# ouguangjun/Leg-KILO

Measured on NVIDIA H100. Metric: LiDAR point-iterations/sec through the ESKF point-to-plane update, higher is better.
Workload: dtype f64

## Files before the change

leg-kilo_b200/csrc/lk_fused.cu:

```cuda
#include "lk_insert.cuh"
#include "lk_kernels.h"
#include "lk_obs.cuh"
#include "lk_pass.cuh"
#include "lk_predict.cuh"
#include "lk_solve.cuh"

namespace lk {

namespace {

#define FT(slot) do { if (a.trace && threadIdx.x == 0 && (slot) < 32) a.trace[(size_t)blockIdx.x * 32 + (slot)] = gtime(); } while (0)
#define FTI(slot) do { if (it_global < 3) FT(slot); } while (0)
#define FTS(slot) do { if (a.trace && blockIdx.x == 0 && threadIdx.x == 0 && k < 64) a.trace[(size_t)gridDim.x * 32 + (size_t)k * 8 + (slot)] = gtime(); } while (0)
#ifndef LK_HOP_TRACE
#define LK_HOP_TRACE 0
#endif
#define FT_HOPS() ((LK_HOP_TRACE && a.trace && it_global < 3) \
                       ? a.trace + (size_t)gridDim.x * 32 + 64 * 8 + (size_t)blockIdx.x * 16 + it_global * LL_HOP_SLOTS : nullptr)

constexpr int BLOCK = FB;
constexpr int WARPS = BLOCK / 32;

struct PredictScratch {
    double F[900];
    double T[900];
    double Ps[900];
    ObsScratch obs;
};

template <bool HOT>
struct FusedSmemT {
    BlockFilter f;
    ScanConst sc;
    double slice[WARPS * 32];
    double clk[2];
    union {
        PredictScratch pr;
        PassSmem<BLOCK, HOT> pass;
    } u;
};
typedef FusedSmemT<true> FusedSmem;

struct FusedSmemIns {
    FusedSmemT<false> base;
    WarpTile wt[WARPS];
    MapDev md;
    Globals g;
};

__device__ __noinline__ void fused_insert_phase2(FusedSmemIns* si, const uint32_t* touched, const int* iroot, const DevPoint* ipts,
                                                 int* pend, uint32_t n_touched, uint32_t n_bucket) {
    const int lane = threadIdx.x & 31, warp = threadIdx.x >> 5;
    MapDev md = si->md;
    WarpTile* wt = si->wt + warp;
    for (uint32_t t = blockIdx.x * (uint32_t)WARPS + (uint32_t)warp; t < n_touched; t += gridDim.x * (uint32_t)WARPS)
        warp_insert_root_scan(md, si->g, wt, __ldcg(&touched[t]), iroot, ipts, n_bucket, pend, lane);
}

static_assert(sizeof(PredictScratch) <= sizeof(((PassSmem<BLOCK, true>*)0)->tile) &&
                  sizeof(PredictScratch) <= sizeof(((PassSmem<BLOCK, false>*)0)->tile),
              "predict scratch must not reach the mbarriers");
static_assert(sizeof(FusedSmemIns) <= 227 * 1024, "one block per SM");
static_assert(sizeof(FusedSmem) + 1024 <= 132 * 1024, "the batch-of-one kernel's stack frames must fit in L1");

int carveout_percent(size_t smem, int dev) {
    int per_sm = 0, per_block = 0;
    cudaDeviceGetAttribute(&per_sm, cudaDevAttrMaxSharedMemoryPerMultiprocessor, dev);
    cudaDeviceGetAttribute(&per_block, cudaDevAttrReservedSharedMemoryPerBlock, dev);
    if (per_sm <= 0) return 100;
    const size_t need = smem + (size_t)per_block;
    const int pct = (int)((need * 100 + (size_t)per_sm - 1) / (size_t)per_sm);
    return pct < 100 ? pct : 100;
}

template <class SM>
__device__ __noinline__ void fused_predict(SM* sm, const double* Q, double dtc, double dt) {
    if (dtc != 0.0) {
        build_F(sm->u.pr.F, sm->f.x, dtc);
        cov_predict(sm->f.P, sm->u.pr.F, sm->u.pr.T, sm->u.pr.Ps, Q, dtc);
    }
    if (dt != 0.0) {
        if (threadIdx.x == 0) state_predict(sm->f.x, dt);
    }
    fence_proxy_async();
    __syncthreads();
}

template <class SM>
__device__ __noinline__ void fused_drain_queue(SM* sm, const FusedArgs& a, uint32_t& mi, double t_bucket) {
    bool drained = false;
    while (mi < a.n_meas) {
        const double ts = a.imu ? a.imu[mi].stamp : a.kin[mi].stamp;
        if (!(ts < t_bucket)) break;
        block_predict_to(&sm->f, sm->clk, ts, sm->u.pr.F, sm->u.pr.T, sm->u.pr.Ps, a.Q);
        if (a.imu) block_obs_imu<BLOCK>(&sm->f, &sm->u.pr.obs, a.imu + mi, &a.ecfg, a.gravity, a.acc_norm);
        else block_obs_kinimu<BLOCK>(&sm->f, &sm->u.pr.obs, a.kin + mi, &a.ecfg, a.gravity, a.acc_norm);
        if (threadIdx.x == 0) sm->clk[1] = ts;
        __syncthreads();
        ++mi;
        drained = true;
    }
    if (drained) {
        fence_proxy_async();
        __syncthreads();
    }
}

__device__ __forceinline__ float4 world_out(const double* X, double pix, double piy, double piz, bool updated) {
    float4 o;
    o.x = (float)(X[0] * pix + X[1] * piy + X[2] * piz + X[9]);
    o.y = (float)(X[3] * pix + X[4] * piy + X[5] * piz + X[10]);
    o.z = (float)(X[6] * pix + X[7] * piy + X[8] * piz + X[11]);
    o.w = updated ? 255.0f : 0.0f;
    return o;
}

template <class SM>
__device__ __forceinline__ void store_state(SM* sm, const FusedArgs& a, uint32_t n_eff) {
    const int tid = threadIdx.x;
    if (tid < 36) a.x[(size_t)a.scan * 36 + tid] = sm->f.x[tid];
    if (tid < 2) reinterpret_cast<double*>(a.clk + a.scan)[tid] = sm->clk[tid];
    if (tid == 0) {
        a.n_eff[a.scan] = n_eff;
        *a.status = (*reinterpret_cast<volatile uint32_t*>(a.ll.stall) ? 1u : 0u) | (*reinterpret_cast<volatile uint32_t*>(&lk_stall_note[0]) ? 2u : 0u);
    }
}

typedef PassSmem<BLOCK, true> PassHot;
typedef PassSmem<BLOCK, false> PassNodes;
constexpr size_t FIN_GS_BYTES = (size_t)LL_MAX_GROUPS * 32 * sizeof(double);
constexpr uint32_t FIN_STAGE = (uint32_t)((sizeof(PassHot::tile) - FIN_GS_BYTES) / (3 * sizeof(double)));
static_assert(offsetof(PredictScratch, F) == 0 && offsetof(PassHot, tile) == 0 && offsetof(PassNodes, tile) == 0,
              "the group sums and the staging area start at the tiles");
static_assert(FIN_GS_BYTES + 3 * sizeof(double) * FIN_STAGE <= sizeof(PassHot::tile) &&
                  sizeof(PassHot::tile) <= sizeof(PassNodes::tile) && sizeof(PassHot::tile) <= offsetof(PassHot, bar),
              "the finishers' staging area must stay inside the tiles, clear of the mbarriers");

template <class SM>
__device__ __noinline__ void fused_finish(SM* sm, const FusedArgs& a, const StepInit& in, uint32_t n_chunks, uint32_t it_global,
                                          bool updated, bool dep_waited) {
    const int tid = threadIdx.x;
    const uint32_t fi = blockIdx.x - n_chunks, nf = gridDim.x - n_chunks;
    if (!dep_waited) asm volatile("griddepcontrol.wait;" ::: "memory");
    constexpr int U = 8;
    const uint32_t step = nf * BLOCK;
    const uint32_t first = in.pt_begin + fi * BLOCK + tid;
    double* st = reinterpret_cast<double*>(reinterpret_cast<unsigned char*>(&sm->u) + FIN_GS_BYTES);
    const uint32_t n_pts = first < in.pt_end ? (in.pt_end - first + step - 1) / step : 0u;
    const uint32_t n_st = a.pts_copy ? 0u : min(n_pts, (FIN_STAGE - (uint32_t)tid + BLOCK - 1) / BLOCK);
    for (uint32_t j0 = 0; j0 < n_st; j0 += U) {
        float4 q[U];
#pragma unroll
        for (int u = 0; u < U; ++u)
            if (j0 + u < n_st) q[u] = __ldcg(a.pts + first + (j0 + u) * step);
#pragma unroll
        for (int u = 0; u < U; ++u)
            if (j0 + u < n_st) {
                PointCtx p;
                imu_point(q[u], a.g, p);
                const uint32_t l = (j0 + u) * BLOCK + tid;
                st[l] = p.pix;
                st[FIN_STAGE + l] = p.piy;
                st[2 * FIN_STAGE + l] = p.piz;
            }
    }
    ll_sum_chunk_rows<WARPS>(a.ll, it_global & 1u, a.epoch + it_global, n_chunks, sm->u.pr.F, sm->f.acc);
    FTI(3 + it_global * 4);
    const uint32_t n = block_solve_state(&sm->f);
    FTI(4 + it_global * 4);
    if (n > 0) {
        updated = true;
        if (tid == 0) sm->clk[1] = in.t_bucket;
    }
    for (uint32_t j = 0; j < n_st; ++j) {
        const uint32_t l = j * BLOCK + tid;
        a.world[first + j * step] = world_out(sm->f.x, st[l], st[FIN_STAGE + l], st[2 * FIN_STAGE + l], updated);
    }
    const float4* pts = a.pts;
    if (a.pts_copy) {
        __threadfence();
        pts = a.pts_copy;
    }
    for (uint32_t i0 = first + n_st * step; i0 < in.pt_end; i0 += U * step) {
        float4 q[U];
#pragma unroll
        for (int u = 0; u < U; ++u)
            if (i0 + u * step < in.pt_end) q[u] = __ldcg(pts + i0 + u * step);
#pragma unroll
        for (int u = 0; u < U; ++u)
            if (i0 + u * step < in.pt_end) {
                PointCtx p;
                imu_point(q[u], a.g, p);
                a.world[i0 + u * step] = world_out(sm->f.x, p.pix, p.piy, p.piz, updated);
            }
    }
    FT(20);
    if (n > 0) cov_prep(&sm->f, BLOCK);
    __syncthreads();
    for (uint32_t e = fi * BLOCK + tid; e < 900; e += nf * BLOCK)
        a.P[(size_t)a.scan * 900 + e] = n > 0 ? cov_entry(&sm->f, (int)e) : sm->f.P[e];
    FT(21);
    if (fi == 0) store_state(sm, a, n);
    FT(22);
}

template <bool INL> struct InlineSel { typedef FusedInline type; };
template <> struct InlineSel<false> { typedef FusedNoInline type; };

__device__ __forceinline__ void grid_sync(const FusedArgs& a, uint32_t& sync_idx) {
    __threadfence();
    __syncthreads();
    if (threadIdx.x < 32) (void)ll_allreduce(a.ll, sync_idx & 1u, a.epoch + sync_idx, blockIdx.x, gridDim.x, 0.0, (int)threadIdx.x);
    ++sync_idx;
    __syncthreads();
    __threadfence();
    fence_proxy_async_global();
}

template <bool OBS, bool INL, bool INS>
__global__ void __launch_bounds__(BLOCK, 1) k_scan_fused(const __grid_constant__ FusedArgs a,
                                                         const __grid_constant__ typename InlineSel<INL>::type inl) {
    extern __shared__ __align__(16) unsigned char smem_raw[];
    FusedSmemT<!INS>* sm = reinterpret_cast<FusedSmemT<!INS>*>(smem_raw);
    const int tid = threadIdx.x, lane = tid & 31, warp = tid >> 5;
    const uint32_t scan = a.scan;
    const bool finisher = blockIdx.x + a.finishers >= gridDim.x;
    asm volatile("griddepcontrol.launch_dependents;" ::: "memory");
    FT(0);
    {
        const double* Pin;
        const double* xin;
        const double* cin;
        if constexpr (INL) { Pin = inl.P; xin = inl.x; cin = inl.clk; }
        else { Pin = a.P_in + (size_t)scan * 900; xin = a.x_in + (size_t)scan * 36; cin = reinterpret_cast<const double*>(a.clk_in + scan); }
        if (a.slim_p && !finisher && (a.finishers || blockIdx.x != 0)) {
            if (tid < 180) sm->f.P[(tid / 6) * 30 + tid % 6] = Pin[(tid / 6) * 30 + tid % 6];
        } else {
            for (int e = tid; e < 900; e += BLOCK) sm->f.P[e] = Pin[e];
        }
        if (tid < 36) sm->f.x[tid] = xin[tid];
        if (tid < 2) sm->clk[tid] = cin[tid];
    }
    if constexpr (INS) {
        FusedSmemIns* si = reinterpret_cast<FusedSmemIns*>(smem_raw);
        WarpTile* wt = si->wt + warp;
        if (lane == 0) {
            mbar_init(&wt->bar, 1);
            wt->phase = 0;
        }
        if (tid == 0) si->md = a.md;
        if (tid < (int)(sizeof(Globals) / 4)) reinterpret_cast<uint32_t*>(&si->g)[tid] = reinterpret_cast<const uint32_t*>(&a.g)[tid];
    }
    pass_init(&sm->u.pass);
    FT(1);
    uint32_t n_eff_total = 0;
    uint32_t phase = 0;
    uint32_t it_global = 0;
    uint32_t cslot = 0;
    uint32_t mi = 0;
    bool dep_waited = false;

    for (uint32_t k = 0; k < a.n_steps; ++k) {
        StepInit in;
        if constexpr (INL) in = inl.steps[k];
        else in = a.inits[(size_t)k * a.batch + scan];
        if (!in.active) continue;
        const uint32_t n_chunks = in.chunk_end - in.chunk_begin;
        const uint32_t my_start = in.pt_begin + blockIdx.x * (uint32_t)BLOCK;
        const uint32_t my_count = blockIdx.x < n_chunks ? min((uint32_t)BLOCK, in.pt_end - my_start) : 0u;
        float4 pre = make_float4(0.f, 0.f, 0.f, 0.f);
        if ((uint32_t)tid < my_count) pre = __ldg(a.pts + my_start + tid);
        FTS(0);
        if constexpr (OBS) fused_drain_queue(sm, a, mi, in.t_bucket);
        FTS(1);
        const double dtc = in.t_bucket - sm->clk[1];
        const double dt = in.t_bucket - sm->clk[0];
        if (dtc != 0.0 || dt != 0.0) fused_predict(sm, a.Q, dtc, dt);
        if (tid == 0) sm->clk[0] = in.t_bucket;
        FTS(2);
        bool updated = false, cov_pending = false;
        uint32_t n_last = 0;
        LaneCache lc;
        lc.have = 0;
        const bool more_steps = k + 1 < a.n_steps;
        for (int it = 0; it < a.iters; ++it, ++it_global) {
            scan_const_from(&sm->f, &sm->sc);
            __syncthreads();
            double acc[32];
#pragma unroll
            for (int i = 0; i < 32; ++i) acc[i] = 0.0;
            if (!a.lane_cache && lc.have == 2) lc.have = 1;
            points_pass<BLOCK, INS>(&sm->u.pass, phase, my_count, sm->sc, a.mv, a.g, lc, pre,
                                    [&](uint32_t, const Row& row) { accumulate_row(row, acc); });
            FTI(14 + it_global);
            const double tot = warp_transpose_sum(acc, lane);
            sm->slice[warp * 32 + lane] = tot;
            __syncthreads();
            FTI(2 + it_global * 4);
            if (it == 0) FTS(3);
            const bool last = it == a.iters - 1;
            if (!OBS && !INS && a.finishers && last) {
                if (finisher) {
                    fused_finish(sm, a, in, n_chunks, it_global, updated, dep_waited);
                } else {
                    if (!dep_waited) asm volatile("griddepcontrol.wait;" ::: "memory");
                    if (a.pts_copy) {
                        if ((uint32_t)tid < my_count) a.pts_copy[my_start + tid] = pre;
                        __threadfence();
                        __syncthreads();
                    }
                    if (warp == 0) {
                        double v = 0.0;
#pragma unroll
                        for (int w = 0; w < WARPS; ++w) v += sm->slice[w * 32 + lane];
                        ll_publish_row(a.ll, it_global & 1u, a.epoch + it_global, blockIdx.x, v, lane);
                    }
                }
                FT(31);
                return;
            }
            if (warp == 0) {
                double v = 0.0;
#pragma unroll
                for (int w = 0; w < WARPS; ++w) v += sm->slice[w * 32 + lane];
                if (!dep_waited) {
                    FT(23);
                    asm volatile("griddepcontrol.wait;" ::: "memory");
                    FT(24);
                }
                sm->f.acc[lane] = ll_allreduce(a.ll, it_global & 1u, a.epoch + it_global, blockIdx.x, n_chunks, v, lane, FT_HOPS(),
                                               a.finishers, it_global >= 2);
            }
            dep_waited = true;
            __syncthreads();
            FTI(3 + it_global * 4);
            if (it == 0) FTS(4);
            const uint32_t n = block_solve_state(&sm->f);
            FTI(4 + it_global * 4);
            if (n > 0) {
                updated = true;
                if (tid == 0) sm->clk[1] = in.t_bucket;
                if (last) cov_pending = INS || more_steps || blockIdx.x == 0;
            }
            n_last = n;
        }
        n_eff_total += n_last;
        FTS(5);
        if constexpr (!INS) {
            if ((uint32_t)tid < my_count) a.world[my_start + tid] = world_out(sm->f.x, lc.pix, lc.piy, lc.piz, updated);
            FT(20);
            if (cov_pending) block_cov_update<BLOCK>(&sm->f);
        } else {
            if (cov_pending) block_cov_update<BLOCK>(&sm->f);
            __syncthreads();
            scan_const_from(&sm->f, &sm->sc);
            __syncthreads();
            MapDev md = a.md;
            const uint32_t n_bucket = in.pt_end - in.pt_begin;
            if ((uint32_t)tid < my_count) {
                DevPoint p;
                make_insert_point(lc.pix, lc.piy, lc.piz, lc.pbx, lc.pby, lc.pbz, sm->sc, a.g, p);
                const uint32_t li = my_start + tid - in.pt_begin;
                a.ipts[li] = p;
                float4 o;
                o.x = (float)p.pw[0]; o.y = (float)p.pw[1]; o.z = (float)p.pw[2];
                o.w = updated ? 255.0f : 0.0f;
                a.world[my_start + tid] = o;
                a.iroot[li] = insert_register_point(md, a.g, p, a.pend, a.touched, &a.ins_counters[cslot]);
            }
            grid_sync(a, it_global);
            FTS(6);
            {
                const uint32_t n_touched = __ldcg(&a.ins_counters[cslot]);
                if (blockIdx.x == 0 && tid == 0) a.ins_counters[cslot ^ 1u] = 0;
                fused_insert_phase2(reinterpret_cast<FusedSmemIns*>(smem_raw), a.touched, a.iroot, a.ipts, a.pend, n_touched, n_bucket);
                cslot ^= 1u;
            }
            grid_sync(a, it_global);
            FTS(7);
        }
    }
    FT(30);
    if (blockIdx.x == 0) {
        if (!dep_waited) asm volatile("griddepcontrol.wait;" ::: "memory");
        __syncthreads();
        for (int e = tid; e < 900; e += BLOCK) a.P[(size_t)scan * 900 + e] = sm->f.P[e];
        store_state(sm, a, n_eff_total);
    }
    FT(31);
}

template <bool OBS, bool INL, bool INS>
cudaError_t launch_one(const FusedArgs& a, const FusedInline* inl, uint32_t grid, cudaStream_t s, int mode) {
    auto kern = k_scan_fused<OBS, INL, INS>;
    constexpr size_t SMEM = INS ? sizeof(FusedSmemIns) : sizeof(FusedSmem);
    static PerDeviceOnce once;
    if (once.first()) {
        int dev = 0;
        cudaGetDevice(&dev);
        cudaError_t e = cudaFuncSetAttribute(kern, cudaFuncAttributeMaxDynamicSharedMemorySize, (int)SMEM);
        if (e != cudaSuccess) return e;
        e = cudaFuncSetAttribute(kern, cudaFuncAttributePreferredSharedMemoryCarveout, carveout_percent(SMEM, dev));
        if (e != cudaSuccess) return e;
    }
    typename InlineSel<INL>::type local_inl;
    const typename InlineSel<INL>::type* ip;
    if constexpr (INL) ip = inl;
    else { local_inl.unused = 0; ip = &local_inl; }
    if (mode == FUSED_LAUNCH_COOPERATIVE) {
        void* params[] = {(void*)&a, (void*)ip};
        return cudaLaunchCooperativeKernel((const void*)kern, dim3(grid), dim3(BLOCK), params, SMEM, s);
    }
    cudaLaunchConfig_t cfg = {};
    cfg.gridDim = dim3(grid);
    cfg.blockDim = dim3(BLOCK);
    cfg.dynamicSmemBytes = SMEM;
    cfg.stream = s;
    cudaLaunchAttribute at[1];
    at[0].id = cudaLaunchAttributeProgrammaticStreamSerialization;
    at[0].val.programmaticStreamSerializationAllowed = 1;
    cfg.attrs = at;
    cfg.numAttrs = mode == FUSED_LAUNCH_PDL ? 1 : 0;
    return cudaLaunchKernelEx(&cfg, kern, a, *ip);
}

}

size_t fused_smem_bytes() { return sizeof(FusedSmem); }

int fused_read_stall(uint32_t out[8]) {
    if (cudaMemcpyFromSymbol(out, lk_stall_note, 32) != cudaSuccess) return -1;
    if (out[0]) {
        const uint32_t z[8] = {0, 0, 0, 0, 0, 0, 0, 0};
        cudaMemcpyToSymbol(lk_stall_note, z, 32);
    }
    return 0;
}

int fused_max_blocks(int device) {
    static int cached[64];
    static bool have[64];
    if (device >= 0 && device < 64 && have[device]) return cached[device];
    int sms = 0;
    cudaDeviceGetAttribute(&sms, cudaDevAttrMultiProcessorCount, device);
    int n = sms < LL_MAX_CHUNKS ? sms : LL_MAX_CHUNKS;
    if (device >= 0 && device < 64) { cached[device] = n; have[device] = true; }
    return n;
}

cudaError_t launch_scan_fused(const FusedArgs& a, const FusedInline* inl, uint32_t grid, cudaStream_t s, int mode) {
    const bool obs = a.n_meas > 0;
    if (a.insert) {
        if (inl) return cudaErrorInvalidValue;
        return obs ? launch_one<true, false, true>(a, inl, grid, s, mode) : launch_one<false, false, true>(a, inl, grid, s, mode);
    }
    if (obs) return inl ? launch_one<true, true, false>(a, inl, grid, s, mode) : launch_one<true, false, false>(a, inl, grid, s, mode);
    return inl ? launch_one<false, true, false>(a, inl, grid, s, mode) : launch_one<false, false, false>(a, inl, grid, s, mode);
}

}
```

leg-kilo_b200/csrc/lk_llsync.cuh:

```cuda
#pragma once
#include <cuda_runtime.h>
#include <stdint.h>

#include "lk_async.cuh"

namespace lk {

constexpr int LK_GROUP = 8;
constexpr int LL_ROW = 32;
constexpr int LL_MAX_CHUNKS = 160;
constexpr int LL_MAX_GROUPS = (LL_MAX_CHUNKS + LK_GROUP - 1) / LK_GROUP;
constexpr int LL_REPLICAS = 4;
constexpr int LL_COPIES = LL_REPLICAS + 1;
constexpr int LL_MAX_FINISHERS = 24;

struct LLView {
    ulonglong2* chunk_rows;
    ulonglong2* group_rows;
    uint32_t* stall;
    uint32_t* acks;
};
constexpr size_t LL_ROWS_BYTES = (size_t)2 * (LL_MAX_CHUNKS + LL_COPIES * LL_MAX_GROUPS) * LL_ROW * sizeof(ulonglong2);
constexpr size_t LL_BYTES = LL_ROWS_BYTES + 64 + 2 * LL_MAX_FINISHERS * sizeof(uint32_t);
constexpr uint32_t LL_SPIN_LIMIT = 1u << 23;
constexpr int LL_HOP_SLOTS = 5;

__device__ __forceinline__ void ll_store(ulonglong2* p, double v, uint32_t tag) {
    const unsigned long long b = (unsigned long long)__double_as_longlong(v);
    const unsigned long long t = (unsigned long long)tag << 32;
    const unsigned long long w0 = (b & 0xffffffffull) | t, w1 = (b >> 32) | t;
    asm volatile("st.relaxed.gpu.global.v2.u64 [%0], {%1, %2};" ::"l"(p), "l"(w0), "l"(w1) : "memory");
}

__device__ __forceinline__ void ll_give_up(uint32_t* stall, uint32_t tag, uint32_t r0, uint32_t n, int lane) {
    if (atomicCAS(stall, 0u, 1u) == 0u) {
        stall[1] = blockIdx.x; stall[2] = tag; stall[3] = r0; stall[4] = n; stall[5] = (uint32_t)lane;
        __threadfence();
    }
}

template <int N, bool KEEP, int SPLIT = N>
__device__ __forceinline__ double ll_sum_rows(const ulonglong2* rows, uint32_t r0, uint32_t n, uint32_t tag, int lane,
                                              uint32_t* stall, uint32_t& rounds, double first = 0.0, bool have_first = false,
                                              double* hi = nullptr) {
    static_assert(N <= 32, "one bit per row");
    const ulonglong2* p = rows + (size_t)r0 * LL_ROW + lane;
    unsigned long long w0[N], w1[N];
    const unsigned long long want = ((unsigned long long)tag << 32);
    uint32_t spins = 0;
    if constexpr (!KEEP) {
        bool all;
        do {
#pragma unroll
            for (int k = 0; k < N; ++k)
                if ((uint32_t)k < n && !(have_first && k == 0))
                    asm volatile("ld.relaxed.gpu.global.v2.u64 {%0, %1}, [%2];" : "=l"(w0[k]), "=l"(w1[k]) : "l"(p + (size_t)k * LL_ROW));
            all = true;
#pragma unroll
            for (int k = 0; k < N; ++k)
                if ((uint32_t)k < n && !(have_first && k == 0))
                    all = all && ((w0[k] & 0xffffffff00000000ull) == want) && ((w1[k] & 0xffffffff00000000ull) == want);
            ++spins;
            if (!all && ((spins & 0xfffu) == 0u)) {
                if (spins >= LL_SPIN_LIMIT || *reinterpret_cast<volatile uint32_t*>(stall) != 0u) {
                    ll_give_up(stall, tag, r0, n, lane);
                    break;
                }
            }
        } while (!all);
    } else {
        uint32_t todo = (n >= 32u ? 0xffffffffu : (1u << n) - 1u) & (have_first ? ~1u : ~0u);
        while (true) {
#pragma unroll
            for (int k = 0; k < N; ++k)
                if ((todo >> k) & 1u)
                    asm volatile("ld.relaxed.gpu.global.v2.u64 {%0, %1}, [%2];" : "=l"(w0[k]), "=l"(w1[k]) : "l"(p + (size_t)k * LL_ROW));
#pragma unroll
            for (int k = 0; k < N; ++k)
                if (((todo >> k) & 1u) && ((w0[k] & 0xffffffff00000000ull) == want) && ((w1[k] & 0xffffffff00000000ull) == want))
                    todo &= ~(1u << k);
            ++spins;
            if (todo == 0u) break;
            if ((spins & 0xfffu) == 0u) {
                if (spins >= LL_SPIN_LIMIT || *reinterpret_cast<volatile uint32_t*>(stall) != 0u) {
                    ll_give_up(stall, tag, r0, n, lane);
                    break;
                }
            }
        }
    }
    rounds = spins;
    double s = 0.0;
#pragma unroll
    for (int k = 0; k < SPLIT; ++k)
        if ((uint32_t)k < n) {
            const double v = (have_first && k == 0) ? first : __longlong_as_double((long long)((w0[k] & 0xffffffffull) | (w1[k] << 32)));
            s += v;
        }
    if constexpr (SPLIT < N) {
        double s2 = 0.0;
#pragma unroll
        for (int k = SPLIT; k < N; ++k)
            if ((uint32_t)k < n) s2 += __longlong_as_double((long long)((w0[k] & 0xffffffffull) | (w1[k] << 32)));
        *hi = s2;
    }
    return s;
}

__device__ __forceinline__ void ll_wait_acks(const uint32_t* acks, uint32_t fin, uint32_t tag, int lane, uint32_t* stall) {
    uint32_t spins = 0;
    bool mine = (uint32_t)lane >= fin;
    while (!__all_sync(0xffffffffu, mine)) {
        if (!mine) {
            uint32_t w;
            asm volatile("ld.acquire.gpu.global.u32 %0, [%1];" : "=r"(w) : "l"(acks + lane) : "memory");
            mine = w == tag;
        }
        if ((++spins & 0xfffu) == 0u && (spins >= LL_SPIN_LIMIT || *reinterpret_cast<volatile uint32_t*>(stall) != 0u)) {
            ll_give_up(stall, tag, 0, fin, lane);
            break;
        }
    }
}

__device__ __forceinline__ double ll_allreduce(const LLView& ll, uint32_t parity, uint32_t tag, uint32_t b, uint32_t n_chunks,
                                               double v, int lane, unsigned long long* hops = nullptr, uint32_t fin = 0,
                                               bool acks_due = false) {
    constexpr size_t COPY = (size_t)LL_MAX_GROUPS * LL_ROW;
    ulonglong2* crows = ll.chunk_rows + (size_t)parity * LL_MAX_CHUNKS * LL_ROW;
    ulonglong2* grows = ll.group_rows + (size_t)parity * LL_COPIES * COPY;
    uint32_t* acks = ll.acks + (size_t)parity * LL_MAX_FINISHERS;
    const uint32_t n_groups = (n_chunks + LK_GROUP - 1) / LK_GROUP;
    uint32_t r1 = 0, r2 = 0;
    if (b < n_chunks) {
        if ((b % LK_GROUP) == 0) {
            if (hops && lane == 0) hops[0] = gtime();
            const uint32_t n = min((uint32_t)LK_GROUP, n_chunks - b);
            const double s = ll_sum_rows<LK_GROUP, false>(crows, b, n, tag, lane, ll.stall, r1, v, true);
            if (hops && lane == 0) hops[1] = gtime();
            ulonglong2* g = grows + (size_t)(b / LK_GROUP) * LL_ROW + lane;
            if (fin && acks_due) ll_wait_acks(acks, fin, tag - 2u, lane, ll.stall);
#pragma unroll
            for (int r = 0; r < LL_REPLICAS; ++r) ll_store(g + (size_t)r * COPY, s, tag);
            if (fin) ll_store(g + (size_t)LL_REPLICAS * COPY, s, tag);
            if (hops && lane == 0) hops[2] = gtime();
        } else {
            ll_store(crows + (size_t)b * LL_ROW + lane, v, tag);
            if (hops && lane == 0) hops[0] = gtime();
        }
    }
    const bool finisher = fin && b >= n_chunks;
    const double t = ll_sum_rows<LL_MAX_GROUPS, true>(grows + (size_t)(finisher ? LL_REPLICAS : b % LL_REPLICAS) * COPY, 0, n_groups,
                                                      tag, lane, ll.stall, r2);
    if (finisher) {
        __syncwarp();
        if (lane == 0) asm volatile("st.release.gpu.global.u32 [%0], %1;" ::"l"(acks + (b - n_chunks)), "r"(tag) : "memory");
    }
    if (hops) {
        r1 = __reduce_max_sync(0xffffffffu, r1);
        r2 = __reduce_max_sync(0xffffffffu, r2);
        if (lane == 0) {
            hops[3] = gtime();
            hops[4] = (unsigned long long)r1 | ((unsigned long long)r2 << 32);
        }
    }
    return t;
}

__device__ __forceinline__ void ll_publish_row(const LLView& ll, uint32_t parity, uint32_t tag, uint32_t b, double v, int lane) {
    ll_store(ll.chunk_rows + ((size_t)parity * LL_MAX_CHUNKS + b) * LL_ROW + lane, v, tag);
}

template <int NWARPS>
__device__ __forceinline__ void ll_sum_chunk_rows(const LLView& ll, uint32_t parity, uint32_t tag, uint32_t n_chunks, double* gs,
                                                  double* out) {
    const int tid = threadIdx.x, lane = tid & 31, warp = tid >> 5;
    const ulonglong2* crows = ll.chunk_rows + (size_t)parity * LL_MAX_CHUNKS * LL_ROW;
    const uint32_t n_groups = (n_chunks + LK_GROUP - 1) / LK_GROUP;
    for (uint32_t g = 2u * (uint32_t)warp; g < n_groups; g += 2u * NWARPS) {
        uint32_t rounds;
        double hi;
        gs[g * 32 + lane] = ll_sum_rows<2 * LK_GROUP, true, LK_GROUP>(crows, g * LK_GROUP, min(2u * LK_GROUP, n_chunks - g * LK_GROUP),
                                                                       tag, lane, ll.stall, rounds, 0.0, false, &hi);
        if (g + 1 < n_groups) gs[(g + 1) * 32 + lane] = hi;
    }
    __syncthreads();
    if (tid < 32) {
        double t = 0.0;
        for (uint32_t g = 0; g < n_groups; ++g) t += gs[g * 32 + tid];
        out[tid] = t;
    }
    __syncthreads();
}

}
```

Before: 3.326 billion.

## Spread LL all-reduce polling across all warps with shared-memory scratch

```diff
diff --git a/leg-kilo_b200/csrc/lk_fused.cu b/leg-kilo_b200/csrc/lk_fused.cu
--- a/leg-kilo_b200/csrc/lk_fused.cu
+++ b/leg-kilo_b200/csrc/lk_fused.cu
@@ -204,13 +204,20 @@
     FT(22);
 }
 
+template <class SM>
+__device__ __forceinline__ double* ll_scratch(SM* sm) { return reinterpret_cast<double*>(sm->u.pass.pt); }
+static_assert(sizeof(PassHot::pt) >= LL_XS * sizeof(double) && sizeof(PassNodes::pt) >= LL_XS * sizeof(double) &&
+                  alignof(PointCtx) >= alignof(double),
+              "the all-reduce's scratch must fit in the point contexts");
+
 template <bool INL> struct InlineSel { typedef FusedInline type; };
 template <> struct InlineSel<false> { typedef FusedNoInline type; };
 
-__device__ __forceinline__ void grid_sync(const FusedArgs& a, uint32_t& sync_idx) {
+template <class SM>
+__device__ __forceinline__ void grid_sync(SM* sm, const FusedArgs& a, uint32_t& sync_idx) {
     __threadfence();
     __syncthreads();
-    if (threadIdx.x < 32) (void)ll_allreduce(a.ll, sync_idx & 1u, a.epoch + sync_idx, blockIdx.x, gridDim.x, 0.0, (int)threadIdx.x);
+    (void)ll_allreduce<WARPS>(a.ll, sync_idx & 1u, a.epoch + sync_idx, blockIdx.x, gridDim.x, 0.0, ll_scratch(sm));
     ++sync_idx;
     __syncthreads();
     __threadfence();
@@ -319,8 +326,8 @@
                 FT(31);
                 return;
             }
+            double v = 0.0;
             if (warp == 0) {
-                double v = 0.0;
 #pragma unroll
                 for (int w = 0; w < WARPS; ++w) v += sm->slice[w * 32 + lane];
                 if (!dep_waited) {
@@ -328,9 +335,10 @@
                     asm volatile("griddepcontrol.wait;" ::: "memory");
                     FT(24);
                 }
-                sm->f.acc[lane] = ll_allreduce(a.ll, it_global & 1u, a.epoch + it_global, blockIdx.x, n_chunks, v, lane, FT_HOPS(),
-                                               a.finishers, it_global >= 2);
-            }
+            }
+            const double t = ll_allreduce<WARPS>(a.ll, it_global & 1u, a.epoch + it_global, blockIdx.x, n_chunks, v, ll_scratch(sm),
+                                                 FT_HOPS(), a.finishers, it_global >= 2);
+            if (warp == 0) sm->f.acc[lane] = t;
             dep_waited = true;
             __syncthreads();
             FTI(3 + it_global * 4);
@@ -368,7 +376,7 @@
                 a.world[my_start + tid] = o;
                 a.iroot[li] = insert_register_point(md, a.g, p, a.pend, a.touched, &a.ins_counters[cslot]);
             }
-            grid_sync(a, it_global);
+            grid_sync(sm, a, it_global);
             FTS(6);
             {
                 const uint32_t n_touched = __ldcg(&a.ins_counters[cslot]);
@@ -376,7 +384,7 @@
                 fused_insert_phase2(reinterpret_cast<FusedSmemIns*>(smem_raw), a.touched, a.iroot, a.ipts, a.pend, n_touched, n_bucket);
                 cslot ^= 1u;
             }
-            grid_sync(a, it_global);
+            grid_sync(sm, a, it_global);
             FTS(7);
         }
     }
diff --git a/leg-kilo_b200/csrc/lk_llsync.cuh b/leg-kilo_b200/csrc/lk_llsync.cuh
--- a/leg-kilo_b200/csrc/lk_llsync.cuh
+++ b/leg-kilo_b200/csrc/lk_llsync.cuh
@@ -24,6 +24,10 @@
 constexpr size_t LL_BYTES = LL_ROWS_BYTES + 64 + 2 * LL_MAX_FINISHERS * sizeof(uint32_t);
 constexpr uint32_t LL_SPIN_LIMIT = 1u << 23;
 constexpr int LL_HOP_SLOTS = 5;
+constexpr int LL_XS = (LK_GROUP + LL_MAX_GROUPS + 1) * 32;
+#ifndef LL_POLL_DEPTH
+#define LL_POLL_DEPTH 1
+#endif
 
 __device__ __forceinline__ void ll_store(ulonglong2* p, double v, uint32_t tag) {
     const unsigned long long b = (unsigned long long)__double_as_longlong(v);
@@ -39,53 +43,30 @@
     }
 }
 
-template <int N, bool KEEP, int SPLIT = N>
+template <int N, int SPLIT = N>
 __device__ __forceinline__ double ll_sum_rows(const ulonglong2* rows, uint32_t r0, uint32_t n, uint32_t tag, int lane,
-                                              uint32_t* stall, uint32_t& rounds, double first = 0.0, bool have_first = false,
-                                              double* hi = nullptr) {
+                                              uint32_t* stall, uint32_t& rounds, double* hi = nullptr) {
     static_assert(N <= 32, "one bit per row");
     const ulonglong2* p = rows + (size_t)r0 * LL_ROW + lane;
     unsigned long long w0[N], w1[N];
     const unsigned long long want = ((unsigned long long)tag << 32);
     uint32_t spins = 0;
-    if constexpr (!KEEP) {
-        bool all;
-        do {
-#pragma unroll
-            for (int k = 0; k < N; ++k)
-                if ((uint32_t)k < n && !(have_first && k == 0))
-                    asm volatile("ld.relaxed.gpu.global.v2.u64 {%0, %1}, [%2];" : "=l"(w0[k]), "=l"(w1[k]) : "l"(p + (size_t)k * LL_ROW));
-            all = true;
-#pragma unroll
-            for (int k = 0; k < N; ++k)
-                if ((uint32_t)k < n && !(have_first && k == 0))
-                    all = all && ((w0[k] & 0xffffffff00000000ull) == want) && ((w1[k] & 0xffffffff00000000ull) == want);
-            ++spins;
-            if (!all && ((spins & 0xfffu) == 0u)) {
-                if (spins >= LL_SPIN_LIMIT || *reinterpret_cast<volatile uint32_t*>(stall) != 0u) {
-                    ll_give_up(stall, tag, r0, n, lane);
-                    break;
-                }
-            }
-        } while (!all);
-    } else {
-        uint32_t todo = (n >= 32u ? 0xffffffffu : (1u << n) - 1u) & (have_first ? ~1u : ~0u);
-        while (true) {
-#pragma unroll
-            for (int k = 0; k < N; ++k)
-                if ((todo >> k) & 1u)
-                    asm volatile("ld.relaxed.gpu.global.v2.u64 {%0, %1}, [%2];" : "=l"(w0[k]), "=l"(w1[k]) : "l"(p + (size_t)k * LL_ROW));
-#pragma unroll
-            for (int k = 0; k < N; ++k)
-                if (((todo >> k) & 1u) && ((w0[k] & 0xffffffff00000000ull) == want) && ((w1[k] & 0xffffffff00000000ull) == want))
-                    todo &= ~(1u << k);
-            ++spins;
-            if (todo == 0u) break;
-            if ((spins & 0xfffu) == 0u) {
-                if (spins >= LL_SPIN_LIMIT || *reinterpret_cast<volatile uint32_t*>(stall) != 0u) {
-                    ll_give_up(stall, tag, r0, n, lane);
-                    break;
-                }
+    uint32_t todo = n >= 32u ? 0xffffffffu : (1u << n) - 1u;
+    while (true) {
+#pragma unroll
+        for (int k = 0; k < N; ++k)
+            if ((todo >> k) & 1u)
+                asm volatile("ld.relaxed.gpu.global.v2.u64 {%0, %1}, [%2];" : "=l"(w0[k]), "=l"(w1[k]) : "l"(p + (size_t)k * LL_ROW));
+#pragma unroll
+        for (int k = 0; k < N; ++k)
+            if (((todo >> k) & 1u) && ((w0[k] & 0xffffffff00000000ull) == want) && ((w1[k] & 0xffffffff00000000ull) == want))
+                todo &= ~(1u << k);
+        ++spins;
+        if (todo == 0u) break;
+        if ((spins & 0xfffu) == 0u) {
+            if (spins >= LL_SPIN_LIMIT || *reinterpret_cast<volatile uint32_t*>(stall) != 0u) {
+                ll_give_up(stall, tag, r0, n, lane);
+                break;
             }
         }
     }
@@ -93,10 +74,7 @@
     double s = 0.0;
 #pragma unroll
     for (int k = 0; k < SPLIT; ++k)
-        if ((uint32_t)k < n) {
-            const double v = (have_first && k == 0) ? first : __longlong_as_double((long long)((w0[k] & 0xffffffffull) | (w1[k] << 32)));
-            s += v;
-        }
+        if ((uint32_t)k < n) s += __longlong_as_double((long long)((w0[k] & 0xffffffffull) | (w1[k] << 32)));
     if constexpr (SPLIT < N) {
         double s2 = 0.0;
 #pragma unroll
@@ -105,6 +83,76 @@
         *hi = s2;
     }
     return s;
+}
+
+template <int NWARPS, int RPW, int DEPTH>
+__device__ __forceinline__ uint32_t ll_poll_rows(const ulonglong2* rows, uint32_t r0, uint32_t k0, uint32_t n, uint32_t tag,
+                                                 uint32_t* stall, double* xs) {
+    static_assert(DEPTH == 1 || DEPTH == 2, "one or two rounds in flight");
+    static_assert(NWARPS * RPW <= 32 * 32, "rows per poll");
+    const int lane = threadIdx.x & 31, warp = threadIdx.x >> 5;
+    const ulonglong2* p = rows + (size_t)(r0 + (uint32_t)warp) * LL_ROW + lane;
+    const unsigned long long want = ((unsigned long long)tag << 32);
+    uint32_t todo = 0;
+#pragma unroll
+    for (int j = 0; j < RPW; ++j) {
+        const uint32_t k = (uint32_t)(warp + j * NWARPS);
+        if (k >= k0 && k < n) todo |= 1u << j;
+    }
+    if (todo == 0u) return 0u;
+    unsigned long long a0[RPW], a1[RPW], b0[RPW], b1[RPW];
+    auto issue = [&](unsigned long long* w0, unsigned long long* w1) {
+#pragma unroll
+        for (int j = 0; j < RPW; ++j)
+            if ((todo >> j) & 1u)
+                asm volatile("ld.relaxed.gpu.global.v2.u64 {%0, %1}, [%2];"
+                             : "=l"(w0[j]), "=l"(w1[j]) : "l"(p + (size_t)j * NWARPS * LL_ROW));
+    };
+    auto inspect = [&](const unsigned long long* w0, const unsigned long long* w1) {
+#pragma unroll
+        for (int j = 0; j < RPW; ++j)
+            if (((todo >> j) & 1u) && ((w0[j] & 0xffffffff00000000ull) == want) && ((w1[j] & 0xffffffff00000000ull) == want)) {
+                xs[(size_t)(warp + j * NWARPS) * 32 + lane] = __longlong_as_double((long long)((w0[j] & 0xffffffffull) | (w1[j] << 32)));
+                todo &= ~(1u << j);
+            }
+    };
+    uint32_t spins = 0;
+    auto watchdog = [&]() -> bool {
+        if ((spins & 0xfffu) == 0u && (spins >= LL_SPIN_LIMIT || *reinterpret_cast<volatile uint32_t*>(stall) != 0u)) {
+            ll_give_up(stall, tag, r0 + k0, n - k0, lane);
+            return true;
+        }
+        return false;
+    };
+    if constexpr (DEPTH == 1) {
+        while (true) {
+            issue(a0, a1);
+            inspect(a0, a1);
+            ++spins;
+            if (todo == 0u || watchdog()) break;
+        }
+    } else {
+        const long long c0 = clock64();
+        issue(a0, a1);
+        inspect(a0, a1);
+        ++spins;
+        if (todo != 0u) {
+            const long long c1 = clock64(), half = (c1 - c0) >> 1;
+            issue(a0, a1);
+            while (clock64() - c1 < half) {}
+            while (true) {
+                issue(b0, b1);
+                inspect(a0, a1);
+                ++spins;
+                if (todo == 0u || watchdog()) break;
+                issue(a0, a1);
+                inspect(b0, b1);
+                ++spins;
+                if (todo == 0u || watchdog()) break;
+            }
+        }
+    }
+    return spins;
 }
 
 __device__ __forceinline__ void ll_wait_acks(const uint32_t* acks, uint32_t fin, uint32_t tag, int lane, uint32_t* stall) {
@@ -123,45 +171,72 @@
     }
 }
 
+template <int NWARPS, int DEPTH = LL_POLL_DEPTH>
 __device__ __forceinline__ double ll_allreduce(const LLView& ll, uint32_t parity, uint32_t tag, uint32_t b, uint32_t n_chunks,
-                                               double v, int lane, unsigned long long* hops = nullptr, uint32_t fin = 0,
+                                               double v, double* xs, unsigned long long* hops = nullptr, uint32_t fin = 0,
                                                bool acks_due = false) {
+    static_assert(LK_GROUP <= NWARPS && 2 * NWARPS <= 64, "one level-1 row per warp; the round counts fit their slots");
+    constexpr int RPW2 = (LL_MAX_GROUPS + NWARPS - 1) / NWARPS;
     constexpr size_t COPY = (size_t)LL_MAX_GROUPS * LL_ROW;
+    const int lane = threadIdx.x & 31, warp = threadIdx.x >> 5;
     ulonglong2* crows = ll.chunk_rows + (size_t)parity * LL_MAX_CHUNKS * LL_ROW;
     ulonglong2* grows = ll.group_rows + (size_t)parity * LL_COPIES * COPY;
     uint32_t* acks = ll.acks + (size_t)parity * LL_MAX_FINISHERS;
+    double* xs1 = xs;
+    double* xs2 = xs + LK_GROUP * 32;
+    uint32_t* rw = reinterpret_cast<uint32_t*>(xs + (LK_GROUP + LL_MAX_GROUPS) * 32);
     const uint32_t n_groups = (n_chunks + LK_GROUP - 1) / LK_GROUP;
     uint32_t r1 = 0, r2 = 0;
     if (b < n_chunks) {
         if ((b % LK_GROUP) == 0) {
-            if (hops && lane == 0) hops[0] = gtime();
+            if (hops && threadIdx.x == 0) hops[0] = gtime();
             const uint32_t n = min((uint32_t)LK_GROUP, n_chunks - b);
-            const double s = ll_sum_rows<LK_GROUP, false>(crows, b, n, tag, lane, ll.stall, r1, v, true);
-            if (hops && lane == 0) hops[1] = gtime();
-            ulonglong2* g = grows + (size_t)(b / LK_GROUP) * LL_ROW + lane;
-            if (fin && acks_due) ll_wait_acks(acks, fin, tag - 2u, lane, ll.stall);
-#pragma unroll
-            for (int r = 0; r < LL_REPLICAS; ++r) ll_store(g + (size_t)r * COPY, s, tag);
-            if (fin) ll_store(g + (size_t)LL_REPLICAS * COPY, s, tag);
-            if (hops && lane == 0) hops[2] = gtime();
-        } else {
+            r1 = ll_poll_rows<NWARPS, 1, DEPTH>(crows, b, 1, n, tag, ll.stall, xs1);
+            __syncthreads();
+            if (warp == 0) {
+                double s = 0.0;
+                s += v;
+#pragma unroll
+                for (uint32_t k = 1; k < (uint32_t)LK_GROUP; ++k)
+                    if (k < n) s += xs1[k * 32 + lane];
+                if (hops && lane == 0) hops[1] = gtime();
+                ulonglong2* g = grows + (size_t)(b / LK_GROUP) * LL_ROW + lane;
+                if (fin && acks_due) ll_wait_acks(acks, fin, tag - 2u, lane, ll.stall);
+#pragma unroll
+                for (int r = 0; r < LL_REPLICAS; ++r) ll_store(g + (size_t)r * COPY, s, tag);
+                if (fin) ll_store(g + (size_t)LL_REPLICAS * COPY, s, tag);
+                if (hops && lane == 0) hops[2] = gtime();
+            }
+        } else if (warp == 0) {
             ll_store(crows + (size_t)b * LL_ROW + lane, v, tag);
             if (hops && lane == 0) hops[0] = gtime();
         }
     }
     const bool finisher = fin && b >= n_chunks;
-    const double t = ll_sum_rows<LL_MAX_GROUPS, true>(grows + (size_t)(finisher ? LL_REPLICAS : b % LL_REPLICAS) * COPY, 0, n_groups,
-                                                      tag, lane, ll.stall, r2);
-    if (finisher) {
-        __syncwarp();
-        if (lane == 0) asm volatile("st.release.gpu.global.u32 [%0], %1;" ::"l"(acks + (b - n_chunks)), "r"(tag) : "memory");
-    }
+    r2 = ll_poll_rows<NWARPS, RPW2, DEPTH>(grows + (size_t)(finisher ? LL_REPLICAS : b % LL_REPLICAS) * COPY, 0, 0, n_groups, tag,
+                                           ll.stall, xs2);
     if (hops) {
         r1 = __reduce_max_sync(0xffffffffu, r1);
         r2 = __reduce_max_sync(0xffffffffu, r2);
         if (lane == 0) {
-            hops[3] = gtime();
-            hops[4] = (unsigned long long)r1 | ((unsigned long long)r2 << 32);
+            rw[2 * warp] = r1;
+            rw[2 * warp + 1] = r2;
+        }
+    }
+    __syncthreads();
+    double t = 0.0;
+    if (warp == 0) {
+        if (finisher && lane == 0) asm volatile("st.release.gpu.global.u32 [%0], %1;" ::"l"(acks + (b - n_chunks)), "r"(tag) : "memory");
+        for (uint32_t g = 0; g < n_groups; ++g) t += xs2[g * 32 + lane];
+        if (hops) {
+            r1 = lane < NWARPS ? rw[2 * lane] : 0u;
+            r2 = lane < NWARPS ? rw[2 * lane + 1] : 0u;
+            r1 = __reduce_max_sync(0xffffffffu, r1);
+            r2 = __reduce_max_sync(0xffffffffu, r2);
+            if (lane == 0) {
+                hops[3] = gtime();
+                hops[4] = (unsigned long long)r1 | ((unsigned long long)r2 << 32);
+            }
         }
     }
     return t;
@@ -180,8 +255,8 @@
     for (uint32_t g = 2u * (uint32_t)warp; g < n_groups; g += 2u * NWARPS) {
         uint32_t rounds;
         double hi;
-        gs[g * 32 + lane] = ll_sum_rows<2 * LK_GROUP, true, LK_GROUP>(crows, g * LK_GROUP, min(2u * LK_GROUP, n_chunks - g * LK_GROUP),
-                                                                       tag, lane, ll.stall, rounds, 0.0, false, &hi);
+        gs[g * 32 + lane] = ll_sum_rows<2 * LK_GROUP, LK_GROUP>(crows, g * LK_GROUP, min(2u * LK_GROUP, n_chunks - g * LK_GROUP),
+                                                                 tag, lane, ll.stall, rounds, &hi);
         if (g + 1 < n_groups) gs[(g + 1) * 32 + lane] = hi;
     }
     __syncthreads();
```

New measurement: 3.479 billion (median of 6 runs). +4.6%, better.
